# kalenforn/clip-based-cross-modal-hash

Hardware: AMD Instinct MI355X
Metric: Hamming query x gallery pairs/sec (fused mAP@all pass, DCMHT COCO-shaped 64-bit) (higher is better)
Workload: dtype u32; 1 GPU; configs[1] DCMHT COCO 64-bit retrieval: Q=5000 queries x R=117218 gallery items per GPU (x1 GPUs, contiguous shards), K=64 bits, C=80 classes, mAP@all; Q=5000, R_per_gpu=117218, K=64, C=80, parallelism=gallery-shard x1, query_blocks=1

## Files before the change

### clip-based-cross-modal-hash_amd/csrc/xmh_scan_kernels.h

```cpp
#pragma once
#include "xmh_scan_mfma.h"

namespace {
template <int W, int LW, bool TERN>
struct QueryRegs {
    uint32_t b[W];
    uint32_t z[TERN ? W : 1];
    uint32_t l[LW];
    __device__ __forceinline__ void load(const ScanArgs& a, int q) {
        const bool ok = q < a.Q;
#pragma unroll
        for (int w = 0; w < W; ++w) b[w] = ok ? a.qbits[(int64_t)q * W + w] : 0u;
        if (TERN) {
#pragma unroll
            for (int w = 0; w < W; ++w) z[w] = ok ? a.qzero[(int64_t)q * W + w] : 0xffffffffu;
        }
#pragma unroll
        for (int w = 0; w < LW; ++w) l[w] = ok ? a.qlab[(int64_t)q * LW + w] : 0u;
    }
};

template <int W, int LW, bool TERN>
struct Rec {
    uint32_t b[W];
// ... 6 lines not shown
    if (!TERN) {
        int acc = 0;
#pragma unroll
        for (int w = 0; w < W; ++w) acc += __popc(qr.b[w] ^ r.b[w]);
        d = acc;
    } else {
        int live_n = 0, diff_n = 0;
#pragma unroll
        for (int w = 0; w < W; ++w) {
            const uint32_t live = ~(qr.z[w] | r.z[w]);
            live_n += __popc(live);
            diff_n += __popc((qr.b[w] ^ r.b[w]) & live);
        }
        d = K - live_n + 2 * diff_n;
    }
    uint32_t hit = qr.l[0] & r.l[0];
#pragma unroll
    for (int w = 1; w < LW; ++w) asm("v_and_or_b32 %0, %1, %2, %0" : "+v"(hit) : "v"(qr.l[w]), "v"(r.l[w]));
    asm("v_min_u32 %0, %1, 1" : "=v"(hit01) : "v"(hit));
}

constexpr uint32_t kRelHi16 = 0xffffffffu;
constexpr int kGateWrapped = 3;
__global__ __launch_bounds__(256) void k_scan_below(const uint32_t* __restrict__ chunk_hist, int qpad, int nb, int nchunk, uint32_t rel_scale,
                                                    uint2* __restrict__ below, uint2* __restrict__ tot, uint32_t* __restrict__ tickets, int Q,
                                                    uint2* __restrict__ dpre, uint32_t* __restrict__ nrel_ws, uint32_t* __restrict__ nrel_max,
                                                    uint32_t* __restrict__ hist_all, uint32_t* __restrict__ hist_rel) {
    __shared__ uint2 part[4][64];
    __shared__ int last;
    const int lane = threadIdx.x & 63, wq = threadIdx.x >> 6;
    const int d = blockIdx.y * 4 + wq;
    const int q = blockIdx.x * 64 + lane;
    const bool hi16 = rel_scale == kRelHi16;
    if (d < nb) {
        uint32_t ra = 0, rr = 0;
        int c = 0;
        for (; c + 4 <= nchunk; c += 4) {
            uint32_t h[4];
#pragma unroll
            for (int j = 0; j < 4; ++j) h[j] = chunk_hist[((int64_t)(c + j) * nb + d) * qpad + q];
#pragma unroll
            for (int j = 0; j < 4; ++j) {
                below[((int64_t)(c + j) * nb + d) * qpad + q] = make_uint2(ra, rr);
                const uint32_t rel = hi16 ? h[j] & 0xffffu : (rel_scale ? h[j] / rel_scale : h[j] >> 16);
                ra += hi16 ? h[j] >> 16 : (rel_scale ? h[j] - rel * rel_scale : h[j] & 0xffffu);
                rr += rel;
            }
        }
        for (; c < nchunk; ++c) {
            const uint32_t h = chunk_hist[((int64_t)c * nb + d) * qpad + q];
            below[((int64_t)c * nb + d) * qpad + q] = make_uint2(ra, rr);
            const uint32_t rel = hi16 ? h & 0xffffu : (rel_scale ? h / rel_scale : h >> 16);
            ra += hi16 ? h >> 16 : (rel_scale ? h - rel * rel_scale : h & 0xffffu);
            rr += rel;
        }
        __hip_atomic_store(reinterpret_cast<unsigned long long*>(tot + (int64_t)d * qpad + q), (unsigned long long)ra | ((unsigned long long)rr << 32),
                           __ATOMIC_RELAXED, __HIP_MEMORY_SCOPE_AGENT);
    }
    if (!tickets) return;
    asm volatile("s_waitcnt vmcnt(0)" ::: "memory");
    __syncthreads();
    if (threadIdx.x == 0) {
        const uint32_t t = __hip_atomic_fetch_add(tickets + blockIdx.x, 1u, __ATOMIC_RELAXED, __HIP_MEMORY_SCOPE_AGENT);
        last = t == gridDim.y - 1;
    }
    __syncthreads();
    if (!last) return;
    auto tot_at = [&](int dd) {
        const unsigned long long v = __hip_atomic_load(reinterpret_cast<const unsigned long long*>(tot + (int64_t)dd * qpad + q), __ATOMIC_RELAXED,
                                                       __HIP_MEMORY_SCOPE_AGENT);
        return make_uint2((uint32_t)v, (uint32_t)(v >> 32));
    };
    const int nbq = (nb + 3) / 4;
    const int d0 = wq * nbq, d1 = (d0 + nbq < nb) ? d0 + nbq : nb;
    uint32_t sa = 0, sr = 0;
    for (int dd = d0; dd < d1; dd += 8) {
        uint2 t[8];
#pragma unroll
        for (int j = 0; j < 8; ++j) t[j] = dd + j < d1 ? tot_at(dd + j) : make_uint2(0u, 0u);
#pragma unroll
        for (int j = 0; j < 8; ++j) { sa += t[j].x; sr += t[j].y; }
    }
    part[wq][lane] = make_uint2(sa, sr);
    __syncthreads();
    uint32_t ra = 0, rr = 0, tr = 0;
#pragma unroll
    for (int w = 0; w < 4; ++w) {
        const uint2 pw = part[w][lane];
        if (w < wq) { ra += pw.x; rr += pw.y; }
        tr += pw.y;
    }
    for (int dd = d0; dd < d1; dd += 8) {
        uint2 t[8];
#pragma unroll
        for (int j = 0; j < 8; ++j) t[j] = dd + j < d1 ? tot_at(dd + j) : make_uint2(0u, 0u);
#pragma unroll
        for (int j = 0; j < 8; ++j) {
            if (dd + j < d1) {
                dpre[(int64_t)(dd + j) * qpad + q] = make_uint2(ra, rr);
                if (hist_all && q < Q) hist_all[(int64_t)q * nb + dd + j] = t[j].x;
                if (hist_rel && q < Q) hist_rel[(int64_t)q * nb + dd + j] = t[j].y;
                ra += t[j].x;
                rr += t[j].y;
            }
        }
    }
    if (wq == 0) {
        nrel_ws[q] = tr;
        if (q < Q) atomicMax(nrel_max, tr);
    }
}

__global__ __launch_bounds__(256) void k_scan_dpre(const uint2* __restrict__ tot, int Q, int qpad, int nb,
                                                   const uint32_t* __restrict__ base_all,
                                                   const uint32_t* __restrict__ base_rel,
                                                   const uint32_t* __restrict__ nrel_total, int64_t kcap,
                                                   uint2* __restrict__ dpre, uint32_t* __restrict__ cap_ws,
                                                   int32_t* __restrict__ cap_out, uint32_t* __restrict__ hist_all,
                                                   uint32_t* __restrict__ hist_rel, uint32_t* __restrict__ nrel_max,
                                                   uint32_t* __restrict__ rank_max = nullptr) {
    __shared__ uint2 part[4][64];
    const int lane = threadIdx.x & 63, wq = threadIdx.x >> 6;
    const int q = blockIdx.x * 64 + lane;
    const bool qok = q < Q;
    const int nbq = (nb + 3) / 4;
    const int d0 = wq * nbq, d1 = (d0 + nbq < nb) ? d0 + nbq : nb;
    uint32_t sa = 0, sr = 0;
    for (int d = d0; d < d1; d += 8) {
        uint2 t[8];
#pragma unroll
        for (int j = 0; j < 8; ++j) t[j] = d + j < d1 ? tot[(int64_t)(d + j) * qpad + q] : make_uint2(0u, 0u);
#pragma unroll
        for (int j = 0; j < 8; ++j) { sa += t[j].x; sr += t[j].y; }
    }
    part[wq][lane] = make_uint2(sa, sr);
    __syncthreads();
    uint32_t ra = 0, rr = 0, ta = 0, tr = 0, rmax = 0;
#pragma unroll
    for (int w = 0; w < 4; ++w) {
        const uint2 p = part[w][lane];
        if (w < wq) { ra += p.x; rr += p.y; }
        ta += p.x; tr += p.y;
// ... 206 lines not shown
        if (CACHE && EB == 8) {
            uint4* dst = crow + ((base - lo) >> 6) * 64;
            __builtin_nontemporal_store(cw0, &dst->x);
            __builtin_nontemporal_store(cw1, &dst->y);
            __builtin_nontemporal_store(cw2, &dst->z);
            __builtin_nontemporal_store(cw3, &dst->w);
        }
        if (CACHE && EB == 16) {
            const uint32_t a0 = (cw0 & 0xfffu) | ((cw0 >> 4) & ~0xfffu), a1 = (cw1 & 0xfffu) | ((cw1 >> 4) & ~0xfffu);
            const uint32_t a2 = (cw2 & 0xfffu) | ((cw2 >> 4) & ~0xfffu), a3 = (cw3 & 0xfffu) | ((cw3 >> 4) & ~0xfffu);
            uint32_t* dst = reinterpret_cast<uint32_t*>(a.pair_cache) +
                            ((((int64_t)chunk_id * a.nqt + qtile) * nbatch + ((base - lo) >> 6)) * 64 + lane) * xmh::kCache12Dwords;
            __builtin_nontemporal_store(a0 | (a1 << 24), dst);
            __builtin_nontemporal_store((a1 >> 8) | (a2 << 16), dst + 1);
            __builtin_nontemporal_store((a2 >> 16) | (a3 << 8), dst + 2);
        }
        cur = nxt;
    }
    uint32_t* __restrict__ out = chunk_hist + ((int64_t)chunk_id * a.nb) * a.qpad + q0;
    for (int e = lane; e < ncell; e += 64) out[(int64_t)(e >> SG::LOG_QW) * a.qpad + (e & (QW - 1))] = cnt[e];
}

template <int W, int LW, bool TERN, bool CAPPED, int S, bool P32, bool MASKED, int NW, bool CACHE>
__global__ __launch_bounds__(64 * NW) void k_scan_ap_s(ScanArgs a, const uint2* __restrict__ below, const uint2* __restrict__ dpre,
                                                  const uint32_t* __restrict__ cap_ws, float* __restrict__ ap_part,
                                                  const uint32_t* __restrict__ nrel_max, int rank_bits, uint32_t kcap,
                                                  const uint32_t* __restrict__ items_total, const uint32_t* __restrict__ run_if = nullptr) {
    using CT = typename std::conditional<P32, uint32_t, unsigned long long>::type;
    extern __shared__ __attribute__((aligned(16))) uint32_t lds[];
    using SG = SlotGeom<S>;
    constexpr int QW = SG::QW, G = SG::G, NG = SG::NG;
    int chunk_id, qtile;
    if (!map_block(a, chunk_id, qtile)) return;
    {
        const bool fits32 = rank_bits > 0 && (uint64_t)(*nrel_max) + 2 < (1ull << (32 - rank_bits));
        if (P32 != fits32) return;
    }
    if (run_if) {
        const bool too_large = items_total && (int64_t)*items_total > kFloatBitsMaxItems;
        if (!too_large && *run_if == 0u) return;
    } else if (items_total && (int64_t)*items_total <= kFloatBitsMaxItems) return;
    const int lane = threadIdx.x & 63, wave = threadIdx.x >> 6;
    const int ql = lane & (QW - 1), slot = lane >> SG::LOG_QW;
    const int q0 = (qtile * NW + wave) * QW;
    const int q = q0 + ql;
    const int ncell = a.nb * QW;
    const int cstride = ((ncell * (int)(sizeof(CT) / 4) + 3) & ~3);
    CT* cnt = reinterpret_cast<CT*>(lds + wave * cstride);
    auto pack = [&](uint2 x, uint2 y) -> CT {
        if (P32) return (CT)((x.x + y.x + 1u) | ((x.y + y.y + 1u) << rank_bits));
        return (CT)((unsigned long long)(x.x + y.x + 1u) | ((unsigned long long)(x.y + y.y + 1u) << 32));
    };
    {
        const uint2* __restrict__ pb = below + ((int64_t)chunk_id * a.nb) * a.qpad + q0;
        const uint2* __restrict__ pd = dpre + q0;
        int e = lane;
        for (; e + 7 * 64 < ncell; e += 8 * 64) {
            uint2 x[8], y[8];
#pragma unroll
            for (int j = 0; j < 8; ++j) {
                const int ee = e + j * 64;
                const int64_t at = (int64_t)(ee >> SG::LOG_QW) * a.qpad + (ee & (QW - 1));
                x[j] = pb[at];
                y[j] = pd[at];
            }
#pragma unroll
// ... 388 lines not shown
    for (int d = d0; d < d1; ++d) {
        uint32_t la = 0, lr = 0;
        for (int w = 0; w < world; ++w) {
            const uint2 t = tot_s[(int64_t)w * plane_in + (int64_t)d * S + s];
            out[(int64_t)w * plane_out + (int64_t)d * S + s] = make_uint2(ra + la, rr + lr);
            la += t.x;
            lr += t.y;
        }
        ra += la;
        rr += lr;
    }
    if (wq == 0)
        for (int w = 0; w < world; ++w) out[(int64_t)w * plane_out + (int64_t)nb * S + s] = make_uint2(tr_all, ta_all);
}

__global__ __launch_bounds__(256) void k_shard_scatter_offsets(const uint2* __restrict__ offs, int nb, int S, int Q, int qpad, int64_t kcap,
                                                               uint2* __restrict__ dpre, uint32_t* __restrict__ cap_ws, int32_t* __restrict__ cap_out,
                                                               uint32_t* __restrict__ items_total) {
    const int q = blockIdx.x * 256 + threadIdx.x;
    if (q >= qpad) return;
    const int owner = q / S, s = q - owner * S;
    const uint2* __restrict__ src = offs + (int64_t)owner * (nb + 1) * S + s;
    const int d = blockIdx.y;
    if (d < nb) {
        dpre[(int64_t)d * qpad + q] = src[(int64_t)d * S];
        return;
    }
    const uint2 t = src[(int64_t)nb * S];
    cap_ws[q] = t.x;
    if (q < Q) cap_out[q] = (int32_t)((kcap > 0 && (uint64_t)kcap < (uint64_t)t.x) ? (uint32_t)kcap : t.x);
    if (q == 0) *items_total = t.y;
}

__device__ __forceinline__ double ap_chunk_sum(const float* __restrict__ ap_part, int qpad, int nchunk, int q, double (*quarter)[64]) {
    const int lane = threadIdx.x & 63, wq = threadIdx.x >> 6;
    const int per = (nchunk + 3) / 4;
    const int c0 = wq * per, c1 = (c0 + per < nchunk) ? c0 + per : nchunk;
    double s = 0.0;
    for (int c = c0; c < c1; c += 8) {
        float v[8];
#pragma unroll
        for (int j = 0; j < 8; ++j) v[j] = c + j < c1 ? ap_part[(int64_t)(c + j) * qpad + q] : 0.0f;
#pragma unroll
        for (int j = 0; j < 8; ++j)
            if (c + j < c1) s += (double)v[j];
    }
    quarter[wq][lane] = s;
    __syncthreads();
    return ((quarter[0][lane] + quarter[1][lane]) + quarter[2][lane]) + quarter[3][lane];
}

__global__ __launch_bounds__(256) void k_ap_reduce(const float* __restrict__ ap_part, int Q, int qpad, int nchunk,
                                                   double* __restrict__ ap_sum, const uint32_t* __restrict__ nrel_ws, uint32_t kcap,
                                                   int32_t* __restrict__ cap_out) {
    __shared__ double quarter[4][64];
    const int q = blockIdx.x * 64 + (threadIdx.x & 63);
    const double s = ap_chunk_sum(ap_part, qpad, nchunk, q, quarter);
    if (threadIdx.x >= 64 || q >= Q) return;
    ap_sum[q] = s;
    if (nrel_ws) cap_out[q] = (int32_t)min(nrel_ws[q], kcap);
}

__global__ __launch_bounds__(256) void k_ap_reduce_map(const float* __restrict__ ap_part, int Q, int qpad, int nchunk,
                                                       const uint32_t* __restrict__ nrel_ws, uint32_t kcap, int32_t* __restrict__ cap_out,
                                                       double* __restrict__ ap_sum, double* __restrict__ part, uint32_t* __restrict__ ticket,
                                                       double* __restrict__ map_out) {
    __shared__ double quarter[4][64];
    __shared__ double red[64];
    __shared__ int last;
    const int lane = threadIdx.x & 63;
    const int q = blockIdx.x * 64 + lane;
    const double s = ap_chunk_sum(ap_part, qpad, nchunk, q, quarter);
    if (threadIdx.x < 64) {
        double term = 0.0;
        if (q < Q) {
            const int32_t cap = (int32_t)min(nrel_ws[q], kcap);
            ap_sum[q] = s;
            cap_out[q] = cap;
            term = s / (double)cap;
        }
        red[lane] = term;
    }
    __syncthreads();
    if (threadIdx.x == 0) {
        double b = 0.0;
        for (int j = 0; j < 64; ++j) b += red[j];
        __hip_atomic_store(&part[blockIdx.x], b, __ATOMIC_RELAXED, __HIP_MEMORY_SCOPE_AGENT);
        asm volatile("s_waitcnt vmcnt(0)" ::: "memory");
        const uint32_t t = __hip_atomic_fetch_add(ticket, 1u, __ATOMIC_RELAXED, __HIP_MEMORY_SCOPE_AGENT);
        last = t == gridDim.x - 1;
    }
    __syncthreads();
    if (!last) return;
    double m = 0.0;
    for (unsigned b0 = 0; b0 < gridDim.x; b0 += 256) {
        const unsigned b = b0 + threadIdx.x;
        __syncthreads();
        reinterpret_cast<double*>(quarter)[threadIdx.x] = b < gridDim.x ? __hip_atomic_load(&part[b], __ATOMIC_RELAXED, __HIP_MEMORY_SCOPE_AGENT) : 0.0;
        __syncthreads();
        if (threadIdx.x == 0) {
            const unsigned n = gridDim.x - b0 < 256u ? gridDim.x - b0 : 256u;
            for (unsigned j = 0; j < n; ++j) m += reinterpret_cast<double*>(quarter)[j];
        }
    }
    if (threadIdx.x == 0) {
// ... 20 lines not shown
```

### clip-based-cross-modal-hash_amd/csrc/xmh_scan_mfma.h

```cpp
#pragma once
#include "xmh_common.h"
#include <type_traits>

namespace {

constexpr int kMaxChunk = 32768;
constexpr uint32_t kF23 = 0x4B000000u;
constexpr int64_t kFloatBitsMaxItems = (1ll << 23) - 3;
constexpr int kMinChunk = 256;

struct ScanArgs {
    const uint32_t* qbits;
    const uint32_t* qzero;
    const uint32_t* qlab;
    const uint32_t* rbits;
    const uint32_t* rzero;
    const uint32_t* rlab;
    int Q, R, K;
    int chunk, nchunk, nqt, qpad, nb;
    uint4* pair_cache;
};

__device__ __forceinline__ bool map_block(const ScanArgs& a, int& chunk_id, int& qtile) {
    const int b = blockIdx.x;
// ... 3 lines not shown
    chunk_id = xcd + 8 * (t / a.nqt);
    return chunk_id < a.nchunk;
}

typedef int v4i __attribute__((ext_vector_type(4)));

struct MfmaArgs {
    const uint32_t* qbits;
    int Q, R, K, W;
    int chunk, nchunk, nqt, nb, qpad;
    const uint32_t* rbits = nullptr;
    const uint32_t* rlab = nullptr;
    const uint32_t* qlab = nullptr;
    int LW = 0;
};

__device__ __forceinline__ bool mfma_map_block(const MfmaArgs& a, int& chunk_id, int& qtile) {
    const int b = blockIdx.x;
    const int xcd = b & 7, t = b >> 3;
    qtile = t % a.nqt;
    chunk_id = xcd + 8 * (t / a.nqt);
    return chunk_id < a.nchunk;
}

__device__ __forceinline__ v4i label_query_f4(uint32_t w, uint32_t one) {
    v4i r;
#pragma unroll
    for (int j = 0; j < 4; ++j) r[j] = (int)(((w >> j) & 0x11111111u) * one);
    return r;
}
__device__ __forceinline__ v4i label_item_f4(uint32_t w) {
    return v4i{(int)(w & 0x11111111u), (int)(w & 0x22222222u), (int)(w & 0x44444444u), (int)((w >> 1) & 0x44444444u)};
}

template <int NML, int NW, int NQ, bool CACHE>
__device__ __forceinline__ void scan_hist_r2_body(const MfmaArgs& a, uint32_t* __restrict__ chunk_hist, uint4* __restrict__ pair_cache) {
    static_assert(NML == 1 || NML == 2, "one i8 label tile (at most 64 classes) or one FP4 label tile (65-128 classes)");
    constexpr bool F4 = NML == 2;
    constexpr int NMI = 2, NMQ = 3;
    constexpr bool REGS = true;
    extern __shared__ __attribute__((aligned(16))) uint32_t lds[];
    int chunk_id, qtile;
    if (!mfma_map_block(a, chunk_id, qtile)) return;
    const int lane = threadIdx.x & 63, wave = threadIdx.x >> 6;
    const int ql = lane & 15, slot = lane >> 4;
    const int t16 = (qtile * NW + wave) * NQ;
    const int ncell = a.nb * 16;
    uint32_t* cnt = lds + (wave * NQ) * ncell;
    for (int e = lane; e < NQ * ncell; e += 64) cnt[e] = 0u;
    v4i bq[NQ][NMQ], cq[NQ], kqv[REGS ? NQ : 1];
    bool valid[NQ];
    const int rsh = 4 * (slot & 1), rwi = slot >> 1;
#pragma unroll
    for (int h = 0; h < NQ; ++h) {
        valid[h] = (t16 + h) * 16 + ql < a.Q;
        int pcq = 0;
        {
            const int64_t q = (int64_t)(t16 + h) * 16 + ql;
            uint32_t qw = 0u;
            if (valid[h]) {
                for (int w = 0; w < a.W; ++w) pcq += __popc(a.qbits[q * a.W + w]);
                if (rwi < a.W) qw = a.qbits[q * a.W + rwi];
            }
            qw >>= rsh;
#pragma unroll
            for (int j = 0; j < 4; ++j) {
                const uint32_t t = (qw >> j) & 0x01010101u;
                const bool on = valid[h] && rwi < a.W;
                if (j & 1) {
                    bq[h][0][j] = on ? (int)(0x20202020u ^ (t * 0xc0u)) : 0;
                    bq[h][1][j] = on ? (int)(0x01010101u ^ (t * 0xfeu)) : 0;
                } else {
                    bq[h][0][j] = on ? (int)(0x40404040u ^ (t << 7)) : 0;
                    bq[h][1][j] = on ? (int)(0x02020202u ^ (t * 0xfcu)) : 0;
                }
            }
            if constexpr (F4) {
                bq[h][2] = label_query_f4(valid[h] && slot < a.LW ? a.qlab[q * a.LW + slot] : 0u, 0x2u);
            } else {
                uint32_t lw = 0u;
                if (valid[h] && rwi < a.LW) lw = a.qlab[q * a.LW + rwi];
                lw >>= rsh;
#pragma unroll
                for (int j = 0; j < 4; ++j) bq[h][2][j] = (int)((lw >> j) & 0x01010101u);
            }
            const int k2 = 2 * pcq;
            kqv[h] = v4i{k2, k2, k2, k2};
        }
        const int c0 = (int)(uint32_t)(uintptr_t)(__attribute__((address_space(3))) uint32_t*)(cnt + h * ncell) + ql * 4 + (valid[h] ? 64 * pcq : 0);
        cq[h] = v4i{c0, c0, c0, c0};
    }
    v4i lab0 = {0x10000, 0x10000, 0x10000, 0x10000};
    asm volatile("" : "+v"(lab0));
#pragma unroll
    for (int h = 0; h < NQ; ++h) asm volatile("" : "+v"(cq[h]));
#pragma unroll
    for (int h = 0; h < (REGS ? NQ : 1); ++h) asm volatile("" : "+v"(kqv[h]));
    const int64_t lo = (int64_t)chunk_id * a.chunk;
    const int64_t hi = (lo + a.chunk < a.R) ? lo + a.chunk : a.R;
    const int nbat = (int)((hi - lo + 63) >> 6);
    const int64_t bat0 = lo >> 6;
    uint4* crow[NQ];
#pragma unroll
    for (int h = 0; h < NQ; ++h)
        crow[h] = CACHE ? pair_cache + ((int64_t)chunk_id * (a.qpad >> 4) + (t16 + h)) * ((a.chunk + 63) >> 6) * 64 + lane : nullptr;
    uint32_t wcur[4][NMI], wnxt[4][NMI];
    const int ritem = 4 * (lane & 3) + ((lane & 15) >> 2);
    const int wi_c = rwi < a.W ? rwi : a.W - 1;
    const int lwi = F4 ? slot : rwi;
    const int wi_l = lwi < a.LW ? lwi : (a.LW > 0 ? a.LW - 1 : 0);
    auto load_words = [&](int64_t batch, uint32_t (&w)[4][NMI]) {
        const int64_t first = batch * 64;
        if (first + 64 <= (int64_t)a.R) {
            const uint32_t* __restrict__ pc = a.rbits + (first + ritem) * a.W + wi_c;
            const uint32_t* __restrict__ pl = a.rlab + (first + ritem) * a.LW + wi_l;
#pragma unroll
            for (int g = 0; g < 4; ++g) {
                w[g][0] = pc[g * 16 * a.W];
                w[g][1] = pl[g * 16 * a.LW];
            }
        } else {
#pragma unroll
            for (int g = 0; g < 4; ++g) {
                const int64_t item = first + g * 16 + ritem;
                const int64_t it = item < a.R ? item : (int64_t)a.R - 1;
                const uint32_t ok = item < a.R ? 0xffffffffu : 0u;
                w[g][0] = a.rbits[it * a.W + wi_c] & ok;
                w[g][1] = a.rlab[it * a.LW + wi_l] & ok;
            }
        }
    };
    auto build = [&](v4i (&At)[NMI], const uint32_t (&w)[NMI]) {
        const uint32_t xa = w[0] >> rsh, xb = w[0] >> (rsh + 2);
        At[0][0] = (int)(xa & 0x01010101u);
        At[0][1] = (int)(xa & 0x02020202u);
        At[0][2] = (int)(xb & 0x01010101u);
        At[0][3] = (int)(xb & 0x02020202u);
        if constexpr (F4) {
// ... 147 lines not shown
            for (int h = 0; h < NQ; ++h) {
                v4i addr, d2, lab;
                if (G == 0 && h == 0) evaluate(A[SET], h, addr, d2, lab);
                else fused(A[SET], h, addr, d2, lab, cw[(h + NQ - 1) % NQ][h == 0 ? G - 1 : G]);
                addr_p = addr; d2_p = d2; lab_p = lab;
                if (REGS && G > 0 && h == 0) {
                    if constexpr (NMI == 2) asm volatile("" ::"v"(A[REGS ? G - 1 : 0][0]), "v"(A[REGS ? G - 1 : 0][1]));
                    else asm volatile("" ::"v"(A[REGS ? G - 1 : 0][0]), "v"(A[REGS ? G - 1 : 0][1]), "v"(A[REGS ? G - 1 : 0][NMI - 1]));
                }
            }
        };
#ifdef XMH_ABL_NOBUILD
        if (i == 0) {
#endif
        build(A[0], wcur[0]);
        build(A[1], wcur[1]);
        build(A[2], wcur[2]);
        build(A[3], wcur[3]);
#ifdef XMH_ABL_NOBUILD
        }
#endif
        group(std::integral_constant<int, 0>{});
        group(std::integral_constant<int, 1>{});
        group(std::integral_constant<int, 2>{});
        group(std::integral_constant<int, 3>{});
        asm volatile(XMH_R2_TAIL ::: "memory");
        consume(cw[NQ - 1][3], A[3]);
#ifdef XMH_ABL_NOSTORE
        if (CACHE && a.Q < 0) {
#else
        if (CACHE) {
#endif
#pragma unroll
            for (int h = 0; h < NQ; ++h) {
                uint4* dst = crow[h] + (int64_t)i * 64;
                __builtin_nontemporal_store(cw[h][0], &dst->x);
                __builtin_nontemporal_store(cw[h][1], &dst->y);
                __builtin_nontemporal_store(cw[h][2], &dst->z);
                __builtin_nontemporal_store(cw[h][3], &dst->w);
            }
        }
#pragma unroll
        for (int g = 0; g < 4; ++g)
#pragma unroll
            for (int m = 0; m < NMI; ++m) wcur[g][m] = wnxt[g][m];
    }
    const int npad = nbat * 64 - (int)(hi - lo);
    asm volatile("s_waitcnt lgkmcnt(0)" ::: "memory");
    if (npad > 0 && slot == 0) {
#pragma unroll
        for (int h = 0; h < NQ; ++h) {
            if (!valid[h]) continue;
            const int64_t q = (int64_t)(t16 + h) * 16 + ql;
            int dpad = 0;
            for (int w = 0; w < a.W; ++w) dpad += __popc(a.qbits[q * a.W + w]);
            cnt[h * ncell + dpad * 16 + ql] -= (uint32_t)npad << 16;
        }
    }
#pragma unroll
    for (int h = 0; h < NQ; ++h) {
        uint32_t* __restrict__ out = chunk_hist + ((int64_t)chunk_id * a.nb) * a.qpad + (t16 + h) * 16;
        for (int e = lane; e < ncell; e += 64) out[(int64_t)(e >> 4) * a.qpad + (e & 15)] = cnt[h * ncell + e];
    }
}

constexpr int kTouchPerChunk = 8;
__global__ __launch_bounds__(256) void k_scan_touch(const uint32_t* __restrict__ rbits, const uint32_t* __restrict__ rlab, int64_t R, int W, int LW, int64_t chunk,
                                                    int nchunk, uint32_t* __restrict__ ctl, int ctl_words) {
    if (blockIdx.x == 0)
        for (int e = threadIdx.x; e < ctl_words; e += 256) ctl[e] = 0u;
    const int b = blockIdx.x;
    const int c = (b & 7) + 8 * ((b >> 3) / kTouchPerChunk), sub = (b >> 3) % kTouchPerChunk;
    if (c >= nchunk) return;
    const int64_t lo = (int64_t)c * chunk, hi = lo + chunk < R ? lo + chunk : R;
    uint32_t acc = 0u;
    auto sweep = [&](const uint32_t* base, int64_t w0, int64_t w1) {
        for (int64_t w = w0 + ((int64_t)sub * 256 + threadIdx.x) * 32; w < w1; w += (int64_t)kTouchPerChunk * 256 * 32) acc ^= base[w];
    };
    sweep(rbits, lo * W, hi * W);
    sweep(rlab, lo * LW, hi * LW);
    asm volatile("" ::"v"(acc));
}

#ifndef XMH_R2_ATTR
#define XMH_R2_ATTR
#endif
template <int NML, int NW, int NQ, bool CACHE>
__global__ __launch_bounds__(64 * NW) XMH_R2_ATTR void k_scan_hist_r2(MfmaArgs a, uint32_t* __restrict__ chunk_hist, uint4* __restrict__ pair_cache) {
    scan_hist_r2_body<NML, NW, NQ, CACHE>(a, chunk_hist, pair_cache);
}

#define XMH_W_MFMA(D, A, B, C) "v_mfma_i32_16x16x64_i8 %[" D "], %[" A "], %[" B "], %[" C "]\n\t"
#define XMH_W_MFMA_F4(D, A, B, C) "v_mfma_f32_16x16x128_f8f6f4 %[" D "], %[" A "], %[" B "], %[" C "] cbsz:4 blgp:4\n\t"
// ... 1 lines not shown
#define XMH_W_ADD(A, D) "ds_add_u32 %[" A "], %[" D "]\n\t"
#define XMH_W_FUSED_CACHE(LAB) \
    asm volatile("s_nop 3\n\t" LAB("lab", "al0", "bl0", "lab0") XMH_W_MIN("i0", "lp0") XMH_W_MIN("i1", "lp1") XMH_W_MIN("i2", "lp2")                \
                 XMH_W_MIN("i3", "lp3") XMH_W_ADD("ap0", "i0") XMH_W_MFMA("addr", "a0", "ba0", "cq") XMH_W_ADD("ap1", "i1")                         \
                 XMH_W_MFMA("addr", "a1", "ba1", "addr") XMH_W_ADD("ap2", "i2") XMH_W_MFMA("d2", "a0", "bd0", "kq") XMH_W_ADD("ap3", "i3")          \
                 XMH_W_MFMA("d2", "a1", "bd1", "d2")                                                                                                \
                 : [lab] "=&v"(lab), [addr] "=&v"(addr), [d2] "=&v"(d2), [i0] "=&v"(i0), [i1] "=&v"(i1), [i2] "=&v"(i2), [i3] "=&v"(i3)             \
                 : [a0] "v"(At[0]), [a1] "v"(At[1]), [al0] "v"(At[2]), [ba0] "v"(bA[h][0]), [ba1] "v"(bA[h][1]), [bd0] "v"(bD[h][0]),               \
                   [bd1] "v"(bD[h][1]), [bl0] "v"(bL[h]), [lab0] "v"(lab0), [cq] "v"(cq[h]), [kq] "v"(kq[h]), [lp0] "v"(lab_p[0]),                  \
                   [lp1] "v"(lab_p[1]), [lp2] "v"(lab_p[2]), [lp3] "v"(lab_p[3]), [ap0] "v"(addr_p[0]), [ap1] "v"(addr_p[1]), [ap2] "v"(addr_p[2]), \
                   [ap3] "v"(addr_p[3])                                                                                                             \
                 : "memory")
#define XMH_W_FUSED_PLAIN(LAB) \
    asm volatile("s_nop 3\n\t" LAB("lab", "al0", "bl0", "lab0") XMH_W_MIN("i0", "lp0") XMH_W_MIN("i1", "lp1") XMH_W_MIN("i2", "lp2")                 \
                 XMH_W_MIN("i3", "lp3") XMH_W_ADD("ap0", "i0") XMH_W_ADD("ap1", "i1") XMH_W_MFMA("addr", "a0", "ba0", "cq") XMH_W_ADD("ap2", "i2")   \
                 XMH_W_ADD("ap3", "i3") XMH_W_MFMA("addr", "a1", "ba1", "addr")                                                                      \
                 : [lab] "=&v"(lab), [addr] "=&v"(addr), [i0] "=&v"(i0), [i1] "=&v"(i1), [i2] "=&v"(i2), [i3] "=&v"(i3)                              \
                 : [a0] "v"(At[0]), [a1] "v"(At[1]), [al0] "v"(At[2]), [ba0] "v"(bA[h][0]), [ba1] "v"(bA[h][1]), [bl0] "v"(bL[h]), [lab0] "v"(lab0), \
                   [cq] "v"(cq[h]), [lp0] "v"(lab_p[0]), [lp1] "v"(lab_p[1]), [lp2] "v"(lab_p[2]), [lp3] "v"(lab_p[3]), [ap0] "v"(addr_p[0]),        \
                   [ap1] "v"(addr_p[1]), [ap2] "v"(addr_p[2]), [ap3] "v"(addr_p[3])                                                                  \
                 : "memory")
template <int NML, int NW, int NQ, bool CACHE>
__global__ __launch_bounds__(64 * NW) void k_scan_hist_r2w(MfmaArgs a, uint32_t* __restrict__ chunk_hist, uint4* __restrict__ pair_cache,
                                                           uint32_t* __restrict__ ovf) {
    static_assert(NML == 1 || NML == 2, "one i8 label tile (at most 64 classes) or one FP4 label tile (65-128 classes)");
    constexpr bool F4 = NML == 2;
    constexpr int NMC = 2, NMI = NMC + 1;
    extern __shared__ __attribute__((aligned(16))) uint32_t lds[];
    int chunk_id, qtile;
    if (!mfma_map_block(a, chunk_id, qtile)) return;
    const int lane = threadIdx.x & 63, wave = threadIdx.x >> 6;
    const int ql = lane & 15, slot = lane >> 4;
    const int t16 = (qtile * NW + wave) * NQ;
    const int ncell = a.nb * 16;
    uint32_t* cnt = lds + (wave * NQ) * ncell;
    for (int e = lane; e < NQ * ncell; e += 64) cnt[e] = 0u;
    const int rsh = 4 * (slot & 1), rwi = slot >> 1;
    v4i bA[NQ][NMC], bD[NQ][NMC], bL[NQ], cq[NQ], kq[NQ];
    bool valid[NQ];
#pragma unroll
    for (int h = 0; h < NQ; ++h) {
        const int64_t q = (int64_t)(t16 + h) * 16 + ql;
        valid[h] = q < a.Q;
        int pcq = 0;
        if (valid[h])
            for (int w = 0; w < a.W; ++w) pcq += __popc(a.qbits[q * a.W + w]);
#pragma unroll
        for (int c = 0; c < NMC; ++c) {
            const int wi = 2 * c + rwi;
            const bool on = valid[h] && wi < a.W;
            const uint32_t qw = (on ? a.qbits[q * a.W + wi] : 0u) >> rsh;
#pragma unroll
            for (int j = 0; j < 4; ++j) {
                const uint32_t t = (qw >> j) & 0x01010101u;
                if (j & 1) {
                    bA[h][c][j] = on ? (int)(0x20202020u ^ (t * 0xc0u)) : 0;
                    bD[h][c][j] = on ? (int)(0x01010101u ^ (t * 0xfeu)) : 0;
                } else {
                    bA[h][c][j] = on ? (int)(0x40404040u ^ (t << 7)) : 0;
                    bD[h][c][j] = on ? (int)(0x02020202u ^ (t * 0xfcu)) : 0;
                }
            }
        }
        if constexpr (F4) {
            bL[h] = label_query_f4(valid[h] && slot < a.LW ? a.qlab[q * a.LW + slot] : 0u, 0x2u);
        } else {
            uint32_t lw = 0u;
            if (valid[h] && rwi < a.LW) lw = a.qlab[q * a.LW + rwi];
            lw >>= rsh;
#pragma unroll
            for (int j = 0; j < 4; ++j) bL[h][j] = (int)((lw >> j) & 0x01010101u);
        }
        const int c0 = (int)(uint32_t)(uintptr_t)(__attribute__((address_space(3))) uint32_t*)(cnt + h * ncell) + ql * 4 + (valid[h] ? 64 * pcq : 0);
        const int k2 = valid[h] ? 2 * pcq : 0;
        cq[h] = v4i{c0, c0, c0, c0};
        kq[h] = v4i{k2, k2, k2, k2};
    }
    v4i lab0 = {0x10000, 0x10000, 0x10000, 0x10000};
    asm volatile("" : "+v"(lab0));
#pragma unroll
    for (int h = 0; h < NQ; ++h) asm volatile("" : "+v"(cq[h]), "+v"(kq[h]));
    const int64_t lo = (int64_t)chunk_id * a.chunk;
    const int64_t hi = (lo + a.chunk < a.R) ? lo + a.chunk : a.R;
    const int nbat = (int)((hi - lo + 63) >> 6);
    const int64_t bat0 = lo >> 6;
    uint4* crow[NQ];
#pragma unroll
    for (int h = 0; h < NQ; ++h)
        crow[h] = CACHE ? pair_cache + ((int64_t)chunk_id * (a.qpad >> 4) + (t16 + h)) * ((a.chunk + 63) >> 6) * 64 + lane : nullptr;
    uint32_t wcur[4][NMI], wnxt[4][NMI];
    const int ritem = 4 * (lane & 3) + ((lane & 15) >> 2);
    int wi_c[NMC];
#pragma unroll
    for (int c = 0; c < NMC; ++c) wi_c[c] = 2 * c + rwi < a.W ? 2 * c + rwi : a.W - 1;
    const int lwi = F4 ? slot : rwi;
    const int wi_l = lwi < a.LW ? lwi : (a.LW > 0 ? a.LW - 1 : 0);
    auto load_words = [&](int64_t batch, uint32_t (&w)[4][NMI]) {
        const int64_t first = batch * 64;
        if (first + 64 <= (int64_t)a.R) {
            const uint32_t* __restrict__ pc = a.rbits + (first + ritem) * a.W;
            const uint32_t* __restrict__ pl = a.rlab + (first + ritem) * a.LW;
#pragma unroll
            for (int g = 0; g < 4; ++g) {
#pragma unroll
                for (int c = 0; c < NMC; ++c) w[g][c] = pc[g * 16 * a.W + wi_c[c]];
                w[g][NMC] = pl[g * 16 * a.LW + wi_l];
            }
        } else {
#pragma unroll
            for (int g = 0; g < 4; ++g) {
                const int64_t item = first + g * 16 + ritem;
                const int64_t it = item < a.R ? item : (int64_t)a.R - 1;
                const uint32_t ok = item < a.R ? 0xffffffffu : 0u;
#pragma unroll
                for (int c = 0; c < NMC; ++c) w[g][c] = a.rbits[it * a.W + wi_c[c]] & ok;
                w[g][NMC] = a.rlab[it * a.LW + wi_l] & ok;
            }
        }
    };
    auto build = [&](v4i (&At)[NMI], const uint32_t (&w)[NMI]) {
#pragma unroll
        for (int c = 0; c < NMC; ++c) {
// ... 70 lines not shown
                if (G == 0 && h == 0) {
                    evaluate(A[G], h, addr, d2, lab);
                } else {
                    uint32_t i0, i1, i2, i3;
                    fused(A[G], h, addr, d2, lab, i0, i1, i2, i3);
                    if (CACHE) pack(cw[(h + NQ - 1) % NQ][h == 0 ? G - 1 : G], d2_p, i0, i1, i2, i3);
                }
                addr_p = addr; d2_p = d2; lab_p = lab;
                if (G > 0 && h == 0) {
                    asm volatile("" ::"v"(A[G > 0 ? G - 1 : 0][0]), "v"(A[G > 0 ? G - 1 : 0][1]), "v"(A[G > 0 ? G - 1 : 0][2]));
                }
            }
        };
        build(A[0], wcur[0]);
        build(A[1], wcur[1]);
        build(A[2], wcur[2]);
        build(A[3], wcur[3]);
        group(std::integral_constant<int, 0>{});
        group(std::integral_constant<int, 1>{});
        group(std::integral_constant<int, 2>{});
        group(std::integral_constant<int, 3>{});
        asm volatile("s_nop 7\n\ts_nop 3" ::: "memory");
        {
            uint32_t i0, i1, i2, i3;
            consume(i0, i1, i2, i3, A[3]);
            if (CACHE) pack(cw[NQ - 1][3], d2_p, i0, i1, i2, i3);
        }
#ifdef XMH_ABL_NOSTORE
        if (CACHE && a.Q < 0) {
#else
        if (CACHE) {
#endif
#pragma unroll
            for (int h = 0; h < NQ; ++h) {
                uint4* dst = crow[h] + (int64_t)i * 64;
                __builtin_nontemporal_store(cw[h][0], &dst->x);
                __builtin_nontemporal_store(cw[h][1], &dst->y);
                __builtin_nontemporal_store(cw[h][2], &dst->z);
                __builtin_nontemporal_store(cw[h][3], &dst->w);
            }
        }
#pragma unroll
        for (int g = 0; g < 4; ++g)
#pragma unroll
            for (int m = 0; m < NMI; ++m) wcur[g][m] = wnxt[g][m];
    }
    const int npad = nbat * 64 - (int)(hi - lo);
    asm volatile("s_waitcnt lgkmcnt(0)" ::: "memory");
    if (npad > 0 && slot == 0) {
#pragma unroll
        for (int h = 0; h < NQ; ++h) {
            if (!valid[h]) continue;
            const int64_t q = (int64_t)(t16 + h) * 16 + ql;
            int dpad = 0;
            for (int w = 0; w < a.W; ++w) dpad += __popc(a.qbits[q * a.W + w]);
            cnt[h * ncell + dpad * 16 + ql] -= (uint32_t)npad << 16;
        }
    }
#pragma unroll
    for (int h = 0; h < NQ; ++h) {
        uint32_t* __restrict__ out = chunk_hist + ((int64_t)chunk_id * a.nb) * a.qpad + (t16 + h) * 16;
        for (int e = lane; e < ncell; e += 64) out[(int64_t)(e >> 4) * a.qpad + (e & 15)] = cnt[h * ncell + e];
    }
    if (CACHE && dmax >= 256u) *ovf = 1u;
}
#undef XMH_W_FUSED_PLAIN
#undef XMH_W_FUSED_CACHE
#undef XMH_W_MFMA_F4
#undef XMH_W_MFMA
#undef XMH_W_MIN
#undef XMH_W_ADD

template <bool CAPPED, int EB, bool HALF = false>
__global__ __launch_bounds__(64) void k_scan_ap_c(ScanArgs a, const uint2* __restrict__ below, const uint2* __restrict__ dpre,
                                                  const uint32_t* __restrict__ cap_ws, float* __restrict__ ap_part,
                                                  const uint32_t* __restrict__ items_total, uint32_t kcap, const uint32_t* __restrict__ skip_if = nullptr,
                                                  const uint32_t* __restrict__ nrel_max = nullptr, int rank_bits = 0) {
    static_assert(!HALF || EB == 8, "the 8 x 8 geometry on one-byte entries");
    constexpr int QW = HALF ? 8 : 128 / EB, LOG_QW = QW == 16 ? 4 : 3, S = 64 / QW, EPW = HALF ? 2 : 32 / EB;
    extern __shared__ __attribute__((aligned(16))) uint32_t lds[];
    int chunk_id, qtile;
    if (!map_block(a, chunk_id, qtile)) return;
    if (items_total && (int64_t)*items_total > kFloatBitsMaxItems) return;
    if (skip_if && *skip_if != 0u) return;
    if (nrel_max && rank_bits > 0 && (uint64_t)(*nrel_max) + 2 < (1ull << (32 - rank_bits))) return;
    const int lane = threadIdx.x & 63;
    const int ql = lane & (QW - 1), slot = lane >> LOG_QW;
    const int q0 = qtile * QW, q = q0 + ql;
    const int ncell = a.nb * QW;
    unsigned long long* cnt = reinterpret_cast<unsigned long long*>(lds);
    {
        const uint2* __restrict__ pb = below + ((int64_t)chunk_id * a.nb) * a.qpad + q0;
        const uint2* __restrict__ pd = dpre + q0;
        auto pack = [](uint2 x, uint2 y) {
            return (unsigned long long)(kF23 + x.x + y.x + 1u) | ((unsigned long long)(kF23 + (0x7fffffu - (x.y + y.y + 1u))) << 32);
        };
        int e = lane;
        for (; e + 7 * 64 < ncell; e += 8 * 64) {
            uint2 x[8], y[8];
#pragma unroll
            for (int j = 0; j < 8; ++j) {
                const int ee = e + j * 64;
                const int64_t at = (int64_t)(ee >> LOG_QW) * a.qpad + (ee & (QW - 1));
                x[j] = pb[at];
                y[j] = pd[at];
            }
#pragma unroll
            for (int j = 0; j < 8; ++j) cnt[e + j * 64] = pack(x[j], y[j]);
        }
        for (; e < ncell; e += 64) {
            const int64_t at = (int64_t)(e >> LOG_QW) * a.qpad + (e & (QW - 1));
            cnt[e] = pack(pb[at], pd[at]);
        }
    }
    const uint32_t cntbase = (uint32_t)(uintptr_t)(__attribute__((address_space(3))) uint32_t*)lds + ql * 8;
// ... 196 lines not shown
    if (slot == 0) ap_part[(int64_t)chunk_id * a.qpad + q] = acc;
}

#define XMH_AP2_SETA "v113", "v115", "v117", "v119", "v[112:113]", "v[114:115]", "v[116:117]", "v[118:119]"
#define XMH_AP2_SETB "v121", "v123", "v125", "v127", "v[120:121]", "v[122:123]", "v[124:125]", "v[126:127]"
#define XMH_AP2_MFMA(D, A, B, C) "v_mfma_i32_16x16x64_i8 %[" D "], %[" A "], %[" B "], " C "\n\t"
#define XMH_AP2_MFMA_F4(D, A, B, C) "v_mfma_f32_16x16x128_f8f6f4 %[" D "], %[" A "], %[" B "], " C " cbsz:4 blgp:4\n\t"
#define XMH_AP2_MAX(H, L) "v_max_i32 " H ", -1, %[" L "]\n\t"
#define XMH_AP2_ADD(O, A, P) "ds_add_rtn_u64 %[" O "], %[" A "], " P "\n\t"
#define XMH_AP2_FUSED_(LAB, H0, H1, H2, H3, P0, P1, P2, P3)                                                                              \
    "s_nop 3\n\t" LAB("lab", "a1", "q1", "0") XMH_AP2_MAX(H0, "l0") XMH_AP2_MAX(H1, "l1") XMH_AP2_MAX(H2, "l2") XMH_AP2_MAX(H3, "l3")    \
    XMH_AP2_MFMA("addr", "a0", "q0", "%[c0]") XMH_AP2_ADD("o0", "p0", P0) XMH_AP2_ADD("o1", "p1", P1) XMH_AP2_ADD("o2", "p2", P2)       \
    XMH_AP2_ADD("o3", "p3", P3)
#define XMH_AP2_TAIL_(H0, H1, H2, H3, P0, P1, P2, P3)                                                                                     \
    XMH_AP2_MAX(H0, "l0") XMH_AP2_MAX(H1, "l1") XMH_AP2_MAX(H2, "l2") XMH_AP2_MAX(H3, "l3") XMH_AP2_ADD("o0", "p0", P0)                   \
    XMH_AP2_ADD("o1", "p1", P1) XMH_AP2_ADD("o2", "p2", P2) XMH_AP2_ADD("o3", "p3", P3)
#define XMH_AP2_FUSED(...) XMH_AP2_FUSED_(__VA_ARGS__)
#define XMH_AP2_TAIL(...) XMH_AP2_TAIL_(__VA_ARGS__)
template <int NML, int NW, int NQ, bool CAPPED>
__global__ __launch_bounds__(64 * NW) void k_scan_ap_r2(MfmaArgs a, const uint2* __restrict__ below, const uint2* __restrict__ dpre,
                                                        const uint32_t* __restrict__ cap_ws, float* __restrict__ ap_part,
                                                        const uint32_t* __restrict__ items_total, uint32_t kcap) {
    using u64 = unsigned long long;
    static_assert(NML == 1 || NML == 2, "one i8 label tile (at most 64 classes) or one FP4 label tile (65-128 classes)");
    constexpr bool F4 = NML == 2;
    constexpr int NMI = 2;
    extern __shared__ __attribute__((aligned(16))) uint32_t lds[];
    int chunk_id, qtile;
    if (!mfma_map_block(a, chunk_id, qtile)) return;
    if (items_total && (int64_t)*items_total > kFloatBitsMaxItems) return;
    const int lane = threadIdx.x & 63, wave = threadIdx.x >> 6;
    const int ql = lane & 15, slot = lane >> 4;
    const int t16 = (qtile * NW + wave) * NQ;
    const int ncell = a.nb * 16;
    u64* cnt = reinterpret_cast<u64*>(lds) + (wave * NQ) * ncell;
    auto pack = [](uint2 x, uint2 y) {
        return (u64)(kF23 + x.x + y.x + 1u) | ((u64)(kF23 + (0x7fffffu - (x.y + y.y + 1u))) << 32);
    };
#pragma unroll
    for (int h = 0; h < NQ; ++h) {
        const uint2* __restrict__ pb = below + ((int64_t)chunk_id * a.nb) * a.qpad + (t16 + h) * 16;
        const uint2* __restrict__ pd = dpre + (t16 + h) * 16;
        u64* c = cnt + h * ncell;
        auto cell = [&](int e) { return e; };
        int e = lane;
        for (; e + 3 * 64 < ncell; e += 4 * 64) {
            uint2 x[4], y[4];
#pragma unroll
            for (int j = 0; j < 4; ++j) {
                const int ee = e + j * 64;
                const int64_t at = (int64_t)(ee >> 4) * a.qpad + (ee & 15);
                x[j] = pb[at];
                y[j] = pd[at];
            }
#pragma unroll
            for (int j = 0; j < 4; ++j) c[cell(e + j * 64)] = pack(x[j], y[j]);
        }
        for (; e < ncell; e += 64) {
            const int64_t at = (int64_t)(e >> 4) * a.qpad + (e & 15);
            c[cell(e)] = pack(pb[at], pd[at]);
        }
    }
    v4i bq[NQ], bl[NQ], cq[NQ];
    float capf[NQ], acc[NQ];
    const int rsh = 4 * (slot & 1), rwi = slot >> 1;
#pragma unroll
// ... 200 lines not shown
```

Measured before the change: 1723 billion pairs/s.

## Skip padded query tiles and route pair-cache stores through bounded buffer resources

Query tiles that lie entirely past Q now exit early in the scan, histogram-write and AP kernels, and padded lanes skip their chunk sums. Pair-cache stores now go through buffer resource descriptors whose size is zero for dead tiles, so hardware bounds checking drops those writes. The stores also use a cache-policy aux bit instead of per-dword nontemporal stores. The chunk prefix walk is fully unrolled at fixed widths of 8, 16, 24 or 32, which issues all loads up front. The aim is to cut wasted memory traffic on padding, at the cost of more code size and extra guard logic.

```diff
diff --git a/clip-based-cross-modal-hash_amd/csrc/xmh_scan_kernels.h b/clip-based-cross-modal-hash_amd/csrc/xmh_scan_kernels.h
--- a/clip-based-cross-modal-hash_amd/csrc/xmh_scan_kernels.h
+++ b/clip-based-cross-modal-hash_amd/csrc/xmh_scan_kernels.h
@@ -62,28 +62,34 @@
     const int d = blockIdx.y * 4 + wq;
     const int q = blockIdx.x * 64 + lane;
     const bool hi16 = rel_scale == kRelHi16;
-    if (d < nb) {
+    if ((int)blockIdx.x * 64 >= Q) return;
+    const bool qok = q < Q;
+    if (d < nb && qok) {
         uint32_t ra = 0, rr = 0;
-        int c = 0;
-        for (; c + 4 <= nchunk; c += 4) {
-            uint32_t h[4];
-#pragma unroll
-            for (int j = 0; j < 4; ++j) h[j] = chunk_hist[((int64_t)(c + j) * nb + d) * qpad + q];
-#pragma unroll
-            for (int j = 0; j < 4; ++j) {
-                below[((int64_t)(c + j) * nb + d) * qpad + q] = make_uint2(ra, rr);
-                const uint32_t rel = hi16 ? h[j] & 0xffffu : (rel_scale ? h[j] / rel_scale : h[j] >> 16);
-                ra += hi16 ? h[j] >> 16 : (rel_scale ? h[j] - rel * rel_scale : h[j] & 0xffffu);
-                rr += rel;
-            }
-        }
-        for (; c < nchunk; ++c) {
-            const uint32_t h = chunk_hist[((int64_t)c * nb + d) * qpad + q];
-            below[((int64_t)c * nb + d) * qpad + q] = make_uint2(ra, rr);
-            const uint32_t rel = hi16 ? h & 0xffffu : (rel_scale ? h / rel_scale : h >> 16);
-            ra += hi16 ? h >> 16 : (rel_scale ? h - rel * rel_scale : h & 0xffffu);
-            rr += rel;
-        }
+        const int64_t cstride = (int64_t)nb * qpad;
+        const uint32_t* __restrict__ src = chunk_hist + (int64_t)d * qpad + q;
+        uint2* __restrict__ dst = below + (int64_t)d * qpad + q;
+        auto walk = [&](int c0, auto nc) {
+            constexpr int N = decltype(nc)::value;
+            uint32_t h[N];
+#pragma unroll
+            for (int j = 0; j < N; ++j) h[j] = src[(int64_t)(c0 + j < nchunk ? c0 + j : nchunk - 1) * cstride];
+#pragma unroll
+            for (int j = 0; j < N; ++j) {
+                if (c0 + j < nchunk) {
+                    dst[(int64_t)(c0 + j) * cstride] = make_uint2(ra, rr);
+                    const uint32_t rel = hi16 ? h[j] & 0xffffu : (rel_scale ? h[j] / rel_scale : h[j] >> 16);
+                    ra += hi16 ? h[j] >> 16 : (rel_scale ? h[j] - rel * rel_scale : h[j] & 0xffffu);
+                    rr += rel;
+                }
+            }
+        };
+        if (nchunk <= 8) walk(0, std::integral_constant<int, 8>{});
+        else if (nchunk <= 16) walk(0, std::integral_constant<int, 16>{});
+        else if (nchunk <= 24) walk(0, std::integral_constant<int, 24>{});
+        else if (nchunk <= 32) walk(0, std::integral_constant<int, 32>{});
+        else
+            for (int c = 0; c < nchunk; c += 16) walk(c, std::integral_constant<int, 16>{});
         __hip_atomic_store(reinterpret_cast<unsigned long long*>(tot + (int64_t)d * qpad + q), (unsigned long long)ra | ((unsigned long long)rr << 32),
                            __ATOMIC_RELAXED, __HIP_MEMORY_SCOPE_AGENT);
     }
@@ -107,12 +113,13 @@
     for (int dd = d0; dd < d1; dd += 8) {
         uint2 t[8];
 #pragma unroll
-        for (int j = 0; j < 8; ++j) t[j] = dd + j < d1 ? tot_at(dd + j) : make_uint2(0u, 0u);
+        for (int j = 0; j < 8; ++j) t[j] = dd + j < d1 && qok ? tot_at(dd + j) : make_uint2(0u, 0u);
 #pragma unroll
         for (int j = 0; j < 8; ++j) { sa += t[j].x; sr += t[j].y; }
     }
     part[wq][lane] = make_uint2(sa, sr);
     __syncthreads();
+    if (!qok) return;
     uint32_t ra = 0, rr = 0, tr = 0;
 #pragma unroll
     for (int w = 0; w < 4; ++w) {
@@ -128,8 +135,8 @@
         for (int j = 0; j < 8; ++j) {
             if (dd + j < d1) {
                 dpre[(int64_t)(dd + j) * qpad + q] = make_uint2(ra, rr);
-                if (hist_all && q < Q) hist_all[(int64_t)q * nb + dd + j] = t[j].x;
-                if (hist_rel && q < Q) hist_rel[(int64_t)q * nb + dd + j] = t[j].y;
+                if (hist_all) hist_all[(int64_t)q * nb + dd + j] = t[j].x;
+                if (hist_rel) hist_rel[(int64_t)q * nb + dd + j] = t[j].y;
                 ra += t[j].x;
                 rr += t[j].y;
             }
@@ -137,7 +144,7 @@
     }
     if (wq == 0) {
         nrel_ws[q] = tr;
-        if (q < Q) atomicMax(nrel_max, tr);
+        atomicMax(nrel_max, tr);
     }
 }
 
@@ -410,6 +417,7 @@
     constexpr int QW = SG::QW, G = SG::G, NG = SG::NG;
     int chunk_id, qtile;
     if (!map_block(a, chunk_id, qtile)) return;
+    if (qtile * NW * QW >= a.Q) return;
     {
         const bool fits32 = rank_bits > 0 && (uint64_t)(*nrel_max) + 2 < (1ull << (32 - rank_bits));
         if (P32 != fits32) return;
@@ -864,10 +872,10 @@
     if (q == 0) *items_total = t.y;
 }
 
-__device__ __forceinline__ double ap_chunk_sum(const float* __restrict__ ap_part, int qpad, int nchunk, int q, double (*quarter)[64]) {
+__device__ __forceinline__ double ap_chunk_sum(const float* __restrict__ ap_part, int Q, int qpad, int nchunk, int q, double (*quarter)[64]) {
     const int lane = threadIdx.x & 63, wq = threadIdx.x >> 6;
     const int per = (nchunk + 3) / 4;
-    const int c0 = wq * per, c1 = (c0 + per < nchunk) ? c0 + per : nchunk;
+    const int c0 = wq * per, c1 = q >= Q ? c0 : ((c0 + per < nchunk) ? c0 + per : nchunk);
     double s = 0.0;
     for (int c = c0; c < c1; c += 8) {
         float v[8];
@@ -887,7 +895,7 @@
                                                    int32_t* __restrict__ cap_out) {
     __shared__ double quarter[4][64];
     const int q = blockIdx.x * 64 + (threadIdx.x & 63);
-    const double s = ap_chunk_sum(ap_part, qpad, nchunk, q, quarter);
+    const double s = ap_chunk_sum(ap_part, Q, qpad, nchunk, q, quarter);
     if (threadIdx.x >= 64 || q >= Q) return;
     ap_sum[q] = s;
     if (nrel_ws) cap_out[q] = (int32_t)min(nrel_ws[q], kcap);
@@ -902,7 +910,7 @@
     __shared__ int last;
     const int lane = threadIdx.x & 63;
     const int q = blockIdx.x * 64 + lane;
-    const double s = ap_chunk_sum(ap_part, qpad, nchunk, q, quarter);
+    const double s = ap_chunk_sum(ap_part, Q, qpad, nchunk, q, quarter);
     if (threadIdx.x < 64) {
         double term = 0.0;
         if (q < Q) {
diff --git a/clip-based-cross-modal-hash_amd/csrc/xmh_scan_mfma.h b/clip-based-cross-modal-hash_amd/csrc/xmh_scan_mfma.h
--- a/clip-based-cross-modal-hash_amd/csrc/xmh_scan_mfma.h
+++ b/clip-based-cross-modal-hash_amd/csrc/xmh_scan_mfma.h
@@ -59,6 +59,30 @@
 __device__ __forceinline__ v4i label_item_f4(uint32_t w) {
     return v4i{(int)(w & 0x11111111u), (int)(w & 0x22222222u), (int)(w & 0x44444444u), (int)((w >> 1) & 0x44444444u)};
 }
+
+constexpr int kCacheStoreAux = 2;
+template <int NQ, bool CACHE>
+struct CacheRows {
+    __amdgpu_buffer_rsrc_t rsrc[CACHE ? NQ : 1];
+    int voff;
+    __device__ __forceinline__ CacheRows(uint4* pair_cache, int64_t first, int rows, int nlive, int lane) : voff(lane * 16) {
+        if constexpr (CACHE) {
+#pragma unroll
+            for (int h = 0; h < NQ; ++h) {
+                const uint64_t base = reinterpret_cast<uint64_t>(pair_cache + first + (int64_t)h * rows);
+                const uint64_t ubase = (uint64_t)(uint32_t)__builtin_amdgcn_readfirstlane((int)(uint32_t)base) |
+                                       ((uint64_t)(uint32_t)__builtin_amdgcn_readfirstlane((int)(uint32_t)(base >> 32)) << 32);
+                rsrc[h] = __builtin_amdgcn_make_buffer_rsrc(reinterpret_cast<void*>(ubase), 0, h < nlive ? rows * 16 : 0, 0x00020000);
+            }
+        }
+    }
+    __device__ __forceinline__ void store(int h, int batch, uint32_t w0, uint32_t w1, uint32_t w2, uint32_t w3) const {
+        if constexpr (CACHE) {
+            typedef uint32_t u32x4_t __attribute__((ext_vector_type(4)));
+            __builtin_amdgcn_raw_buffer_store_b128(u32x4_t{w0, w1, w2, w3}, rsrc[h], voff, batch * 1024, kCacheStoreAux);
+        }
+    }
+};
 
 template <int NML, int NW, int NQ, bool CACHE>
 __device__ __forceinline__ void scan_hist_r2_body(const MfmaArgs& a, uint32_t* __restrict__ chunk_hist, uint4* __restrict__ pair_cache) {
@@ -72,6 +96,7 @@
     const int lane = threadIdx.x & 63, wave = threadIdx.x >> 6;
     const int ql = lane & 15, slot = lane >> 4;
     const int t16 = (qtile * NW + wave) * NQ;
+    const int nlive = __builtin_amdgcn_readfirstlane((a.Q + 15) / 16 - t16);
     const int ncell = a.nb * 16;
     uint32_t* cnt = lds + (wave * NQ) * ncell;
     for (int e = lane; e < NQ * ncell; e += 64) cnt[e] = 0u;
@@ -127,10 +152,7 @@
     const int64_t hi = (lo + a.chunk < a.R) ? lo + a.chunk : a.R;
     const int nbat = (int)((hi - lo + 63) >> 6);
     const int64_t bat0 = lo >> 6;
-    uint4* crow[NQ];
-#pragma unroll
-    for (int h = 0; h < NQ; ++h)
-        crow[h] = CACHE ? pair_cache + ((int64_t)chunk_id * (a.qpad >> 4) + (t16 + h)) * ((a.chunk + 63) >> 6) * 64 + lane : nullptr;
+    CacheRows<NQ, CACHE> crow(pair_cache, ((int64_t)chunk_id * (a.qpad >> 4) + t16) * ((a.chunk + 63) >> 6) * 64, ((a.chunk + 63) >> 6) * 64, nlive, lane);
     uint32_t wcur[4][NMI], wnxt[4][NMI];
     const int ritem = 4 * (lane & 3) + ((lane & 15) >> 2);
     const int wi_c = rwi < a.W ? rwi : a.W - 1;
@@ -344,13 +366,7 @@
         if (CACHE) {
 #endif
 #pragma unroll
-            for (int h = 0; h < NQ; ++h) {
-                uint4* dst = crow[h] + (int64_t)i * 64;
-                __builtin_nontemporal_store(cw[h][0], &dst->x);
-                __builtin_nontemporal_store(cw[h][1], &dst->y);
-                __builtin_nontemporal_store(cw[h][2], &dst->z);
-                __builtin_nontemporal_store(cw[h][3], &dst->w);
-            }
+            for (int h = 0; h < NQ; ++h) crow.store(h, i, cw[h][0], cw[h][1], cw[h][2], cw[h][3]);
         }
 #pragma unroll
         for (int g = 0; g < 4; ++g)
@@ -371,6 +387,7 @@
     }
 #pragma unroll
     for (int h = 0; h < NQ; ++h) {
+        if (h >= nlive) continue;
         uint32_t* __restrict__ out = chunk_hist + ((int64_t)chunk_id * a.nb) * a.qpad + (t16 + h) * 16;
         for (int e = lane; e < ncell; e += 64) out[(int64_t)(e >> 4) * a.qpad + (e & 15)] = cnt[h * ncell + e];
     }
@@ -438,6 +455,7 @@
     const int lane = threadIdx.x & 63, wave = threadIdx.x >> 6;
     const int ql = lane & 15, slot = lane >> 4;
     const int t16 = (qtile * NW + wave) * NQ;
+    const int nlive = __builtin_amdgcn_readfirstlane((a.Q + 15) / 16 - t16);
     const int ncell = a.nb * 16;
     uint32_t* cnt = lds + (wave * NQ) * ncell;
     for (int e = lane; e < NQ * ncell; e += 64) cnt[e] = 0u;
@@ -490,10 +508,7 @@
     const int64_t hi = (lo + a.chunk < a.R) ? lo + a.chunk : a.R;
     const int nbat = (int)((hi - lo + 63) >> 6);
     const int64_t bat0 = lo >> 6;
-    uint4* crow[NQ];
-#pragma unroll
-    for (int h = 0; h < NQ; ++h)
-        crow[h] = CACHE ? pair_cache + ((int64_t)chunk_id * (a.qpad >> 4) + (t16 + h)) * ((a.chunk + 63) >> 6) * 64 + lane : nullptr;
+    CacheRows<NQ, CACHE> crow(pair_cache, ((int64_t)chunk_id * (a.qpad >> 4) + t16) * ((a.chunk + 63) >> 6) * 64, ((a.chunk + 63) >> 6) * 64, nlive, lane);
     uint32_t wcur[4][NMI], wnxt[4][NMI];
     const int ritem = 4 * (lane & 3) + ((lane & 15) >> 2);
     int wi_c[NMC];
@@ -630,13 +645,7 @@
         if (CACHE) {
 #endif
 #pragma unroll
-            for (int h = 0; h < NQ; ++h) {
-                uint4* dst = crow[h] + (int64_t)i * 64;
-                __builtin_nontemporal_store(cw[h][0], &dst->x);
-                __builtin_nontemporal_store(cw[h][1], &dst->y);
-                __builtin_nontemporal_store(cw[h][2], &dst->z);
-                __builtin_nontemporal_store(cw[h][3], &dst->w);
-            }
+            for (int h = 0; h < NQ; ++h) crow.store(h, i, cw[h][0], cw[h][1], cw[h][2], cw[h][3]);
         }
 #pragma unroll
         for (int g = 0; g < 4; ++g)
@@ -657,6 +666,7 @@
     }
 #pragma unroll
     for (int h = 0; h < NQ; ++h) {
+        if (h >= nlive) continue;
         uint32_t* __restrict__ out = chunk_hist + ((int64_t)chunk_id * a.nb) * a.qpad + (t16 + h) * 16;
         for (int e = lane; e < ncell; e += 64) out[(int64_t)(e >> 4) * a.qpad + (e & 15)] = cnt[h * ncell + e];
     }
@@ -679,6 +689,7 @@
     extern __shared__ __attribute__((aligned(16))) uint32_t lds[];
     int chunk_id, qtile;
     if (!map_block(a, chunk_id, qtile)) return;
+    if (qtile * QW >= a.Q) return;
     if (items_total && (int64_t)*items_total > kFloatBitsMaxItems) return;
     if (skip_if && *skip_if != 0u) return;
     if (nrel_max && rank_bits > 0 && (uint64_t)(*nrel_max) + 2 < (1ull << (32 - rank_bits))) return;
@@ -941,6 +952,7 @@
     const int lane = threadIdx.x & 63, wave = threadIdx.x >> 6;
     const int ql = lane & 15, slot = lane >> 4;
     const int t16 = (qtile * NW + wave) * NQ;
+    if (t16 * 16 >= a.Q) return;
     const int ncell = a.nb * 16;
     u64* cnt = reinterpret_cast<u64*>(lds) + (wave * NQ) * ncell;
     auto pack = [](uint2 x, uint2 y) {
```

Measured after the change: 1739 billion pairs/s (median of 6 runs). About the same (+1.0%).
